# rust-av/grav1synth

Measured on AMD Instinct MI355X. Metric: diff Mpixels/s (luma pixels of frame pairs fully processed: flat-block finder + AR accumulation + block stats + ordered fold), higher is better.
Workload: dtype i8 x i8 -> i32 matrix-core products, i64 sums (exact integers) + f64 flat-block features

## Files before the change

grav1synth_amd/csrc/latest.hip:

```cpp
#include "latest_dev.h"

#include "fold.h"

#include <stdio.h>

namespace g1s {
namespace {

constexpr int kT = 512, kWaves = kT / 64;
constexpr int kChunk = 1024, kRounds = kChunk / kT;
constexpr double kTinyD = 1.0e-16;
constexpr double kNorm2D = 255.0 * 255.0;
constexpr int kNL = 2 * kNumBins;
constexpr int kArenaD = 2 * kChunk + 8 * kNumBins + 8, kArenaL = kChunk + 8 * kNumBins + 8, kArenaT = kChunk + 8;
static_assert(kNumBins == 20 && kMaxN == 25, "latest.hip: the solvers' static sizes");

struct Shared {
  alignas(16) double D[kArenaD];
  double Lw[kArenaL];
  double Bv[2][kArenaD];
  double Tv[2][kArenaT];
  uint16_t cnt[kRounds][kWaves][kNL];
  uint32_t beg[kNL], end[kNL];
  double arx[3][kMaxN + 1];
  double gain[3];
  long long nobs[3];
  int ar_ok[3];
  double diag[kNumBins], low[kNumBins], bsum[2][kNumBins], total[2];
  double sb[2][kNumBins], sx[2][kNumBins];
  int st_ok[2];
  double luma_x[kNumBins];
  uint32_t ne;
  uint32_t wsum[kWaves];
};

__device__ __forceinline__ double readlane_f64(double v, int j) {
  const unsigned long long u = (unsigned long long)__double_as_longlong(v);
  const uint32_t lo = (uint32_t)__builtin_amdgcn_readlane((int)(uint32_t)u, j), hi = (uint32_t)__builtin_amdgcn_readlane((int)(uint32_t)(u >> 32), j);
  return __longlong_as_double((long long)(((unsigned long long)hi << 32) | lo));
}
__device__ __forceinline__ int uniform(int v) { return __builtin_amdgcn_readfirstlane(v); }

template <int NMAX>
__device__ __forceinline__ bool wave_gauss(const int n, double (&a)[NMAX], double b, double (&x)[NMAX], const int lane) {
  int rap = lane;
  bool done = false, ok = true;
#pragma unroll
  for (int k = 0; k < NMAX - 1; ++k) {
    if (k < n - 1 && ok) {
      const double ck = fabs(a[k]);
      double cp = __shfl(ck, rap, 64);
      if (lane < k || lane >= n) cp = -1.0;
      double val = cp;
      int idx = lane;
#pragma unroll
      for (int d = 1; d < 32; d <<= 1) {
        const double v2 = __shfl_down(val, d, 64);
        const int i2 = __shfl_down(idx, d, 64);
        if (lane + d < 64 && v2 > val) {
          val = v2;
          idx = i2;
        }
      }
      const int rap_w = __shfl(rap, idx, 64);
      const int rap_up = __shfl_up(rap, 1, 64);
      const double cp_up = __shfl_up(cp, 1, 64);
      if (lane >= k && lane < n) rap = (lane == k) ? rap_w : ((cp_up < val) ? rap_up : rap_w);
      const int pr = uniform(__shfl(rap, k, 64));
      const double pk = readlane_f64(a[k], pr), bk = readlane_f64(b, pr);
      if (fabs(pk) < kTinyD) {
        ok = false;
      } else {
        if (lane == pr) done = true;
        const bool active = lane < n && !done;
        const double c = a[k] / pk;
#pragma unroll
        for (int j = k + 1; j < NMAX; ++j) {
          const double pj = readlane_f64(a[j], pr);
          const double t = c * pj;
          if (active && j < n) a[j] = a[j] - t;
        }
        const double t = c * bk;
        if (active) b = b - t;
      }
    }
  }
#pragma unroll
  for (int i = NMAX - 1; i >= 0; --i) {
    if (i < n && ok) {
      const int r = uniform(__shfl(rap, i, 64));
      const double piv = readlane_f64(a[i], r);
      if (fabs(piv) < kTinyD) {
        ok = false;
      } else {
        double c = 0;
#pragma unroll
        for (int j = i + 1; j < NMAX; ++j) {
          const double t = a[j] * x[j];
          if (j < n) c += t;
        }
        const double xi = (b - c) / a[i];
        x[i] = __shfl(xi, r, 64);
      }
    }
  }
  return ok;
}

__device__ inline double dev_clamp(double v, double lo, double hi) { return v < lo ? lo : (v > hi ? hi : v); }
__device__ inline double dev_bin_index(double value) { return (kNumBins - 1) * dev_clamp(value, 0.0, 255.0) / 255.0; }

__device__ __forceinline__ double div_count(double v, int count) {
  return (count & (count - 1)) == 0 ? __builtin_ldexp(v, -__builtin_ctz((unsigned)count)) : v / count;
}

__device__ inline void put_text(char *dst, const char *msg) {
  int i = 0;
  for (; msg[i] && i < 103; ++i) dst[i] = msg[i];
  dst[i] = 0;
}

#ifdef G1S_LATEST_TIMERS
#define K4_TICK(slot)                                 \
  do {                                                \
    __syncthreads();                                  \
    if (tid == 0 && frame == 0) {                     \
      const unsigned long long now_ = wall_clock64(); \
      k4_dbg[slot] += (double)(now_ - k4_t);          \
      k4_t = now_;                                    \
    }                                                 \
  } while (0)
#else
#define K4_TICK(slot) \
  do {                \
  } while (0)
#endif

struct FrameCtx {
  const uint8_t *rec;
  const uint8_t *mask;
  const uint32_t *luma_sum;
  int nb, nbw, W, H;
};

template <int NP>
__device__ __forceinline__ void strength_pass(Shared &sh, const LatestJob &job, const FrameCtx &fc, const int c0, const int tid, double *k4_dbg, const int frame) {
#ifdef G1S_LATEST_TIMERS
  unsigned long long k4_t = wall_clock64();
#endif
  const int lane = tid & 63, wave = tid >> 6;
  const bool is_chroma = c0 != 0;
  const int sx = is_chroma ? job.xdec : 0, sy = is_chroma ? job.ydec : 0;
  const int bw = kBlock >> sx, bh = kBlock >> sy;
  const int pw = job.W >> sx, ph = job.H >> sy;
  const int32_t *sum_d[NP];
  const uint32_t *sum_d2[NP];
  double noise_gain[NP], corr[NP];
#pragma unroll
  for (int q = 0; q < NP; ++q) {
    sum_d[q] = reinterpret_cast<const int32_t *>(fc.rec + job.L.off_sum_d[c0 + q]);
    sum_d2[q] = reinterpret_cast<const uint32_t *>(fc.rec + job.L.off_sum_d2[c0 + q]);
    noise_gain[q] = sh.gain[c0 + q];
    corr[q] = is_chroma ? sh.arx[c0 + q][job.n] : 0;
  }
  const double luma_gain = sh.gain[0];
  double acc = 0;
  uint32_t ne = 0;

  struct Raw {
    uint32_t m, ls;
    int32_t sd[NP];
    uint32_t sd2[NP];
  };
  Raw nxt[kRounds];
  auto fetch = [&](int base) {
#pragma unroll
    for (int r = 0; r < kRounds; ++r) {
      const int bi = base + kT * r + tid;
      const bool in = bi < fc.nb;
      nxt[r].m = in ? fc.mask[bi] : 0u;
      nxt[r].ls = in ? fc.luma_sum[bi] : 0u;
#pragma unroll
      for (int q = 0; q < NP; ++q) {
        nxt[r].sd[q] = in ? sum_d[q][bi] : 0;
        nxt[r].sd2[q] = in ? sum_d2[q][bi] : 0u;
      }
    }
  };
  fetch(0);
  for (int base = 0; base < fc.nb; base += kChunk) {
    Raw cur[kRounds];
#pragma unroll
    for (int r = 0; r < kRounds; ++r) cur[r] = nxt[r];
    if (base + kChunk < fc.nb) fetch(base + kChunk);
    int key[kRounds];
    double tU[kRounds], tW[kRounds], tV[kRounds], tP[kRounds][NP], tQ[kRounds][NP], tS[kRounds][NP];
#pragma unroll
    for (int r = 0; r < kRounds; ++r) {
      const int bi = base + kT * r + tid;
      key[r] = -1;
      tU[r] = tW[r] = tV[r] = 0;
#pragma unroll
      for (int q = 0; q < NP; ++q) tP[r][q] = tQ[r][q] = tS[r][q] = 0;
      if (cur[r].m == 0) continue;
      const int by = bi / fc.nbw, bx = bi - by * fc.nbw;
      const int shh = min(ph - by * bh, bh), sw = min(pw - bx * bw, bw);
      if (!(sw * shh > kBlock)) continue;
      const int lw = min(fc.W - bx * kBlock, kBlock), lh = min(fc.H - by * kBlock, kBlock);
      const double block_mean = div_count((double)cur[r].ls, lw * lh);
      const double bin = dev_bin_index(block_mean);
      const int i0 = (int)bin;
      const int i1 = min(kNumBins - 1, i0 + 1);
      const double a = bin - i0;
      key[r] = i0;
      tU[r] = (1.0 - a) * (1.0 - a);
      tW[r] = a * (1.0 - a);
      tV[r] = a * a;
      const double luma_strength = is_chroma ? luma_gain * ((1.0 - a) * sh.luma_x[i0] + a * sh.luma_x[i1]) : 0;
#pragma unroll
      for (int q = 0; q < NP; ++q) {
        double noise_mean = (double)cur[r].sd[q];
        const double noise_sq = (double)cur[r].sd2[q];
        noise_mean = div_count(noise_mean, sw * shh);
        const double noise_var = div_count(noise_sq, sw * shh) - noise_mean * noise_mean;
        const double cl = corr[q] * luma_strength;
        const double t0 = noise_var / 16, t1 = noise_var - cl * cl;
        const double uncorr_std = sqrt(t0 > t1 ? t0 : t1);
        const double noise_std = uncorr_std / noise_gain[q];
        tS[r][q] = noise_std;
        tP[r][q] = (1.0 - a) * noise_std;
        tQ[r][q] = a * noise_std;
      }
    }
    K4_TICK(6);
    uint32_t rk_own[kRounds], rk_prev[kRounds], rk_low[kRounds], rk_all[kRounds];
#pragma unroll
    for (int r = 0; r < kRounds; ++r) {
      unsigned long long prevB = 0;
      uint32_t mycnt = 0;
      rk_own[r] = rk_prev[r] = rk_low[r] = rk_all[r] = 0;
      const int kk = key[r];
#pragma unroll
      for (int k = 0; k < kNumBins; ++k) {
        const unsigned long long Bk = __ballot(kk == k);
        const unsigned long long M = Bk | prevB;
        if (M == 0) continue;
        const uint32_t preM = __builtin_amdgcn_mbcnt_hi((uint32_t)(M >> 32), __builtin_amdgcn_mbcnt_lo((uint32_t)M, 0u));
        const uint32_t preB = __builtin_amdgcn_mbcnt_hi((uint32_t)(Bk >> 32), __builtin_amdgcn_mbcnt_lo((uint32_t)Bk, 0u));
        if (kk == k) rk_own[r] = preM, rk_low[r] = preB;
        if (kk == k - 1) rk_prev[r] = preM;
        if (lane == k) mycnt = (uint32_t)__popcll(M);
        if (lane == kNumBins + k) mycnt = (uint32_t)__popcll(Bk);
        prevB = Bk;
      }
      {
        const unsigned long long Ma = __ballot(kk >= 0);
        rk_all[r] = __builtin_amdgcn_mbcnt_hi((uint32_t)(Ma >> 32), __builtin_amdgcn_mbcnt_lo((uint32_t)Ma, 0u));
        if (lane == kNL - 1) mycnt = (uint32_t)__popcll(Ma);
      }
      if (lane < kNL) sh.cnt[r][wave][lane] = (uint16_t)mycnt;
    }
    __syncthreads();
    K4_TICK(7);
    uint32_t my_off[kRounds];
    uint32_t run = 0;
#pragma unroll
    for (int r = 0; r < kRounds; ++r) my_off[r] = 0;
    if (lane < kNL) {
#pragma unroll
      for (int r = 0; r < kRounds; ++r)
#pragma unroll
        for (int w = 0; w < kWaves; ++w) {
          if (w == wave) my_off[r] = run;
          run += sh.cnt[r][w][lane];
        }
    }
    {
      const uint32_t room = (run + 7u) & ~7u;
      uint32_t incl = room;
#pragma unroll
      for (int d = 1; d < 64; d <<= 1) {
        const uint32_t o = (uint32_t)__shfl_up((int)incl, d, 64);
        if (lane >= d) incl += o;
      }
      const uint32_t upto19 = (uint32_t)__shfl((int)incl, kNumBins - 1, 64);
      uint32_t bse = incl - room;
      if (lane >= kNumBins) bse -= upto19;
      if (lane == kNL - 1) bse = 0;
#pragma unroll
      for (int r = 0; r < kRounds; ++r) my_off[r] += bse;
      if (wave == 0 && lane < kNL) {
        sh.beg[lane] = bse;
        sh.end[lane] = bse + run;
        if (lane < kNumBins) {
          for (uint32_t i = bse + run; i < bse + room; ++i) {
            sh.D[i] = 0.0;
#pragma unroll
            for (int q = 0; q < NP; ++q) sh.Bv[q][i] = 0.0;
          }
        } else if (lane < kNL - 1) {
          for (uint32_t i = bse + run; i < bse + room; ++i) sh.Lw[i] = 0.0;
        } else {
          for (uint32_t i = run; i < room; ++i) {
#pragma unroll
            for (int q = 0; q < NP; ++q) sh.Tv[q][i] = 0.0;
          }
        }
      }
    }
    K4_TICK(8);
#pragma unroll
    for (int r = 0; r < kRounds; ++r) {
      const int kk = key[r], kq = max(kk, 0);
      const uint32_t o_own = (uint32_t)__shfl((int)my_off[r], kq, 64);
      const uint32_t o_prev = (uint32_t)__shfl((int)my_off[r], min(kq + 1, kNumBins - 1), 64);
      const uint32_t o_low = (uint32_t)__shfl((int)my_off[r], kNumBins + min(kq, kNumBins - 2), 64);
      const uint32_t o_all = (uint32_t)__shfl((int)my_off[r], kNL - 1, 64);
      if (kk < 0) continue;
      const uint32_t so = o_own + rk_own[r];
      sh.D[so] = tU[r];
#pragma unroll
      for (int q = 0; q < NP; ++q) sh.Bv[q][so] = tP[r][q];
      if (kk < kNumBins - 1) {
        const uint32_t sp = o_prev + rk_prev[r];
        sh.D[sp] = tV[r];
#pragma unroll
        for (int q = 0; q < NP; ++q) sh.Bv[q][sp] = tQ[r][q];
        const uint32_t sl = o_low + rk_low[r];
        sh.Lw[sl] = tW[r];
      }
      const uint32_t st = o_all + rk_all[r];
#pragma unroll
      for (int q = 0; q < NP; ++q) sh.Tv[q][st] = tS[r][q];
    }
    __syncthreads();
    K4_TICK(9);
    if (wave == 0 || wave == 2) {
      constexpr int kLowLanes = kNumBins - 1;
      const int arr = wave == 0 ? lane / kNumBins : (lane < kLowLanes ? 3 : 4 + (lane - kLowLanes));
      const int li = wave == 0 ? lane % kNumBins : (lane < kLowLanes ? kNumBins + lane : kNL - 1);
      const bool on = wave == 0 ? arr <= NP : lane < kLowLanes + NP;
      const double2 *src = reinterpret_cast<const double2 *>(arr == 0 ? sh.D : arr == 1 ? sh.Bv[0] : arr == 2 ? sh.Bv[NP - 1] : arr == 3 ? sh.Lw : arr == 4 ? sh.Tv[0] : sh.Tv[NP - 1]);
      if (on) {
        uint32_t i = sh.beg[li] >> 1;
        const uint32_t e = (sh.end[li] + 1) >> 1;
        double2 va[4], vb[4];
#pragma unroll
        for (int u = 0; u < 4; ++u) va[u] = src[i + u];
        while (i < e) {
#pragma unroll
          for (int u = 0; u < 4; ++u) vb[u] = src[i + 4 + u];
#pragma unroll
          for (int u = 0; u < 4; ++u) acc += va[u].x, acc += va[u].y;
          i += 4;
          if (i < e) {
#pragma unroll
            for (int u = 0; u < 4; ++u) va[u] = src[i + 4 + u];
#pragma unroll
            for (int u = 0; u < 4; ++u) acc += vb[u].x, acc += vb[u].y;
            i += 4;
          }
        }
        if (wave == 2 && lane == kLowLanes) ne += sh.end[kNL - 1];
      }
    }
    __syncthreads();
    K4_TICK(10);
  }
  if (wave == 0) {
    const int k = lane % kNumBins, arr = lane / kNumBins;
    if (arr == 0) sh.diag[k] = acc;
    else if (arr <= NP) sh.bsum[arr - 1][k] = acc;
  } else if (wave == 2) {
    if (lane < kNumBins - 1) sh.low[lane] = acc;
    else if (lane < kNumBins - 1 + NP) sh.total[lane - (kNumBins - 1)] = acc;
    if (lane == kNumBins - 1) sh.ne = ne;
  }
  __syncthreads();
}

__device__ __forceinline__ void strength_solve(Shared &sh, const int q, const int lane) {
  const uint32_t ne = sh.ne;
  double r[kNumBins], x[kNumBins];
  const int i = lane < kNumBins ? lane : 0, nn = kNumBins;
  const double mean = sh.total[q] / (int)ne;
  const double sb = sh.bsum[q][i] + mean / 8192.;
  const double alpha = 2.0 * (double)(int)ne / nn;
  const int lo = max(0, i - 1), hi = min(nn - 1, i + 1);
#pragma unroll
  for (int j = 0; j < kNumBins; ++j) {
    double v = 0.0;
    if (i == j) v = sh.diag[i];
    else if (i == j + 1) v = sh.low[j];
    else if (j == i + 1) v = sh.low[i];
    r[j] = v;
    x[j] = 0.0;
  }
#pragma unroll
  for (int j = 0; j < kNumBins; ++j)
    if (j == lo) r[j] -= alpha;
#pragma unroll
  for (int j = 0; j < kNumBins; ++j)
    if (j == i) r[j] += 2 * alpha;
#pragma unroll
  for (int j = 0; j < kNumBins; ++j)
    if (j == hi) r[j] -= alpha;
#pragma unroll
  for (int j = 0; j < kNumBins; ++j)
    if (j == i) r[j] += 1.0 / 8192.;
  const bool ok = wave_gauss<kNumBins>(kNumBins, r, sb, x, lane);
  if (lane < kNumBins) {
    sh.sb[q][lane] = sb;
    double xv = 0.0;
#pragma unroll
    for (int j = 0; j < kNumBins; ++j)
      if (j == lane) xv = x[j];
    sh.sx[q][lane] = xv;
  }
  if (lane == 0) sh.st_ok[q] = ok ? 1 : 0;
}

__global__ __launch_bounds__(kT) void k4_latest(LatestJob job) {
  __shared__ Shared sh;
  const int tid = threadIdx.x, lane = tid & 63, wave = tid >> 6, frame = blockIdx.x;
  const uint8_t *rec = job.records + job.L.size * (size_t)frame;
  uint8_t *blob = job.blobs + job.blob_bytes * (size_t)frame;
  const int nb = (int)job.L.nblocks;
  const int n = job.n, ncm = n + 1;
  FrameCtx fc;
  fc.rec = rec;
  fc.mask = rec + job.L.off_mask;
  fc.luma_sum = reinterpret_cast<const uint32_t *>(rec + job.L.off_luma_sum);
  fc.nb = nb;
  fc.nbw = job.nbw;
  fc.W = job.W;
  fc.H = job.H;

  double *k4_dbg = reinterpret_cast<double *>(job.scratch);
#ifdef G1S_LATEST_TIMERS
  unsigned long long k4_t = wall_clock64();
  if (tid < 16 && frame == 0) k4_dbg[tid] = 0.0;
  __syncthreads();
#endif
  for (size_t k = tid; k < job.blob_bytes / 8; k += kT) reinterpret_cast<unsigned long long *>(blob)[k] = 0ull;
  LatestHeader *hdr = reinterpret_cast<LatestHeader *>(blob);
  auto plane_head = [&](int c) { return reinterpret_cast<LatestPlaneHead *>(blob + sizeof(LatestHeader) + c * plane_blob_bytes(ncm)); };
  auto plane_doubles = [&](int c) { return reinterpret_cast<double *>(blob + sizeof(LatestHeader) + c * plane_blob_bytes(ncm) + sizeof(LatestPlaneHead)); };
  uint32_t nflat_t = 0;
  for (int b = tid; b < nb; b += kT) nflat_t += fc.mask[b] != 0;
#pragma unroll
  for (int d = 32; d > 0; d >>= 1) nflat_t += (uint32_t)__shfl_down((int)nflat_t, d, 64);
  if (lane == 0) sh.wsum[wave] = nflat_t;
  __syncthreads();
  uint32_t num_flat = 0;
#pragma unroll
  for (int w = 0; w < kWaves; ++w) num_flat += sh.wsum[w];
  if (tid == 0) {
    hdr->magic = kLatestMagic;
    hdr->lag = (uint32_t)job.lag;
    hdr->nplanes = (uint32_t)job.nplanes;
    hdr->status = G1S_OK;
    hdr->size_bytes = (uint32_t)job.blob_bytes;
    hdr->reserved = num_flat;
    for (int c = 0; c < 3; ++c) plane_head(c)->ar_gain = 1.0;
  }
  if (num_flat <= 1) {
    if (tid == 0) {
      hdr->status = G1S_ERR_NOT_ENOUGH_FLAT;
      put_text(hdr->err, "Not enough flat blocks to update noise estimate");
    }
    return;
  }
  K4_TICK(0);

  auto ar_entry = [&](int c, int i, int j) -> double {
    const bool is_chroma = c != 0;
    const int nc = n + (is_chroma ? 1 : 0);
    const int64_t *S = reinterpret_cast<const int64_t *>(rec + job.L.off_ar[c]);
    const double ns = is_chroma ? (double)((1 << job.xdec) * (1 << job.ydec)) : 1.0;
    double den = kNorm2D;
    if (is_chroma && i == nc - 1) den *= ns;
    if (is_chroma && j == nc - 1) den *= ns;
    const int64_t s = j == nc ? S[(size_t)nc * nc + i] : (i <= j ? S[i * nc + j] : S[j * nc + i]);
    return (double)s / den;
  };
  if (wave < job.nplanes) {
    const int c = wave;
    const bool is_chroma = c != 0;
    const int nc = n + (is_chroma ? 1 : 0);
    const int row = lane < nc ? lane : 0;
    double a[kMaxN], x[kMaxN];
#pragma unroll
    for (int j = 0; j < kMaxN; ++j) {
      a[j] = j < nc ? ar_entry(c, row, j) : 0.0;
      x[j] = 0.0;
    }
    const double b0 = ar_entry(c, row, nc);
    const double a_diag = ar_entry(c, row, row), a_last = ar_entry(c, row, nc - 1);
    const int64_t nobs = reinterpret_cast<const int64_t *>(rec + job.L.off_ar[c])[(size_t)nc * nc + nc];
    const bool ok = wave_gauss<kMaxN>(nc, a, b0, x, lane);
    double gain = 1.0;
    if (ok) {
      const int m = nc - (is_chroma ? 1 : 0);
      double x_mine = 0.0;
#pragma unroll
      for (int j = 0; j < kMaxN; ++j)
        if (j == lane) x_mine = x[j];
      const double tv = a_diag / nobs;
      double bi = b0, x_last = 0.0;
#pragma unroll
      for (int j = 0; j < kMaxN; ++j)
        if (j == nc - 1) x_last = x[j];
      if (is_chroma) bi -= a_last * x_last;
      const double tc = (bi * x_mine) / nobs;
      double var = 0, sum_covar = 0;
      for (int i = 0; i < m; ++i) var += readlane_f64(tv, i);
      var /= m;
      for (int i = 0; i < m; ++i) sum_covar += readlane_f64(tc, i);
      const double t = var - sum_covar;
      const double noise_var = t > 1e-6 ? t : 1e-6;
      const double q = var / noise_var;
      const double g = sqrt(q > 1e-6 ? q : 1e-6);
      gain = 1 > g ? 1 : g;
    } else if (is_chroma) {
      const int last = nc - 1;
      const double all = readlane_f64(a_diag, last), bl = readlane_f64(b0, last);
#pragma unroll
      for (int j = 0; j < kMaxN; ++j) x[j] = 0.0;
      if (fabs(all) > 1e-6) {
        const double xl = bl / all;
#pragma unroll
        for (int j = 0; j < kMaxN; ++j)
          if (j == last) x[j] = xl;
      }
    }
    if (lane < nc) {
      double xv = 0.0;
#pragma unroll
      for (int j = 0; j < kMaxN; ++j)
        if (j == lane) xv = x[j];
      sh.arx[c][lane] = xv;
    }
    if (lane == 0) {
      sh.gain[c] = gain;
      sh.nobs[c] = nobs;
      sh.ar_ok[c] = ok ? 1 : 0;
    }
  }
  __syncthreads();
  K4_TICK(1);
  auto write_ar = [&](int c) {
    const bool is_chroma = c != 0;
    const int nc = n + (is_chroma ? 1 : 0);
    double *pd = plane_doubles(c);
    for (int e = tid; e < nc * nc + nc; e += kT) {
      if (e < nc * nc) {
        const int i = e / nc, j = e - i * nc;
        pd[e] = ar_entry(c, i, j);
      } else {
        const int i = e - nc * nc;
        pd[ncm * ncm + i] = ar_entry(c, i, nc);
        pd[ncm * ncm + ncm + i] = sh.arx[c][i];
      }
    }
    if (tid == 0) {
      LatestPlaneHead *ph = plane_head(c);
      ph->num_observations = sh.nobs[c];
      ph->ar_gain = sh.gain[c];
    }
  };
  auto write_strength = [&](int c, int q) {
    double *qd = plane_doubles(c) + ncm * ncm + 2 * ncm;
    for (int e = tid; e < kNumBins * kNumBins; e += kT) {
      const int i = e / kNumBins, j = e - i * kNumBins;
      double v = 0.0;
      if (i == j) v = sh.diag[i];
      else if (i == j + 1) v = sh.low[j];
      else if (j == i + 1) v = sh.low[i];
      qd[e] = v;
    }
    if (tid < kNumBins) {
      qd[kNumBins * kNumBins + tid] = sh.sb[q][tid];
      qd[kNumBins * kNumBins + kNumBins + tid] = sh.sx[q][tid];
    }
    if (tid == 0) {
      LatestPlaneHead *ph = plane_head(c);
      ph->num_equations = (int32_t)sh.ne;
      ph->total = sh.total[q];
    }
  };
  write_ar(0);
  if (!sh.ar_ok[0]) {
    if (tid == 0) {
      hdr->status = G1S_ERR_SOLVE;
      put_text(hdr->err, "Solving latest noise equation system failed 0!");
    }
    return;
  }
  strength_pass<1>(sh, job, fc, 0, tid, k4_dbg, frame);
  K4_TICK(2);
  if (wave == 0) strength_solve(sh, 0, lane);
  __syncthreads();
  write_strength(0, 0);
  if (tid < kNumBins) sh.luma_x[tid] = sh.sx[0][tid];
  if (!sh.st_ok[0]) {
    if (tid == 0) {
      hdr->status = G1S_ERR_SOLVE;
      put_text(hdr->err, "Solving latest noise strength failed!");
    }
    return;
  }
  __syncthreads();
  K4_TICK(3);
  if (job.nplanes < 3) return;
  strength_pass<2>(sh, job, fc, 1, tid, k4_dbg, frame);
  K4_TICK(4);
  if (wave < 2) strength_solve(sh, wave, lane);
  __syncthreads();
  write_ar(1);
  write_strength(1, 0);
  if (!sh.st_ok[0]) {
    if (tid == 0) {
      hdr->status = G1S_ERR_SOLVE;
      put_text(hdr->err, "Solving latest noise strength failed!");
    }
    return;
  }
  write_ar(2);
  write_strength(2, 1);
  if (!sh.st_ok[1]) {
    if (tid == 0) {
      hdr->status = G1S_ERR_SOLVE;
      put_text(hdr->err, "Solving latest noise strength failed!");
    }
  }
  K4_TICK(5);
}

}

size_t latest_scratch_bytes(uint32_t) { return 256; }
const char *latest_kernel_name() { return "k4_latest"; }

hipError_t launch_latest(const LatestJob &job, int frames, hipStream_t stream) {
  if (frames <= 0) return hipSuccess;
  hipLaunchKernelGGL(k4_latest, dim3(frames), dim3(kT), 0, stream, job);
#ifdef G1S_LATEST_TIMERS
  {
    double t[16];
    (void)hipStreamSynchronize(stream);
    (void)hipMemcpy(t, job.scratch, sizeof(t), hipMemcpyDeviceToHost);
    fprintf(stderr, "k4_latest phases, us (frame 0): head %.1f  ar solves %.1f  luma pass %.1f  luma solve %.1f  chroma pass %.1f  chroma solves %.1f | inside both passes: "
                    "terms %.1f  ranks %.1f  offsets %.1f  scatter %.1f  chains %.1f\n",
            t[0] / 100, t[1] / 100, t[2] / 100, t[3] / 100, t[4] / 100, t[5] / 100, t[6] / 100, t[7] / 100, t[8] / 100, t[9] / 100, t[10] / 100);
  }
#endif
  return hipGetLastError();
}

}
```

Baseline: 657,200.

## Pipeline strength pass with dedicated chain waves and double-buffered arenas; DPP pivot search

Splits the block into 8 producer waves and 2 extra high-priority chain waves. Producers compute terms and ranks for stage t+2 and scatter stage t+1 into double-buffered shared arenas while the chain waves sum stage t, so each stage needs one barrier instead of two. The stage size drops from 1024 to 512 blocks. The Gaussian pivot argmax now uses DPP row shifts and readlane in place of shfl_down/shfl, which caps the system size at 32. The cost is more threads per block, a larger shared-memory footprint, and more pipeline stages for the same work.

```diff
diff --git a/grav1synth_amd/csrc/latest.hip b/grav1synth_amd/csrc/latest.hip
--- a/grav1synth_amd/csrc/latest.hip
+++ b/grav1synth_amd/csrc/latest.hip
@@ -7,21 +7,24 @@
 namespace g1s {
 namespace {
 
-constexpr int kT = 512, kWaves = kT / 64;
-constexpr int kChunk = 1024, kRounds = kChunk / kT;
+constexpr int kPT = 512, kPW = kPT / 64;
+constexpr int kCW = 2;
+constexpr int kT = kPT + 64 * kCW, kWaves = kT / 64;
+constexpr int kStage = 512, kRounds = kStage / kPT;
 constexpr double kTinyD = 1.0e-16;
 constexpr double kNorm2D = 255.0 * 255.0;
 constexpr int kNL = 2 * kNumBins;
-constexpr int kArenaD = 2 * kChunk + 8 * kNumBins + 8, kArenaL = kChunk + 8 * kNumBins + 8, kArenaT = kChunk + 8;
+constexpr int kArenaD = 2 * kStage + 8 * kNumBins + 8, kArenaL = kStage + 8 * kNumBins + 8, kArenaT = kStage + 8;
 static_assert(kNumBins == 20 && kMaxN == 25, "latest.hip: the solvers' static sizes");
+static_assert(kArenaD % 2 == 0 && kArenaL % 2 == 0 && kArenaT % 2 == 0, "latest.hip: the chains read the arenas as double2");
 
 struct Shared {
-  alignas(16) double D[kArenaD];
-  double Lw[kArenaL];
-  double Bv[2][kArenaD];
-  double Tv[2][kArenaT];
-  uint16_t cnt[kRounds][kWaves][kNL];
-  uint32_t beg[kNL], end[kNL];
+  alignas(16) double D[2][kArenaD];
+  double Lw[2][kArenaL];
+  double Bv[2][2][kArenaD];
+  double Tv[2][2][kArenaT];
+  uint16_t cnt[2][kRounds][kPW][kNL];
+  uint32_t beg[2][kNL], end[2][kNL];
   double arx[3][kMaxN + 1];
   double gain[3];
   long long nobs[3];
@@ -39,10 +42,30 @@
   const uint32_t lo = (uint32_t)__builtin_amdgcn_readlane((int)(uint32_t)u, j), hi = (uint32_t)__builtin_amdgcn_readlane((int)(uint32_t)(u >> 32), j);
   return __longlong_as_double((long long)(((unsigned long long)hi << 32) | lo));
 }
-__device__ __forceinline__ int uniform(int v) { return __builtin_amdgcn_readfirstlane(v); }
+
+template <int CTRL>
+__device__ __forceinline__ int dpp_i32(int old, int v) {
+  return __builtin_amdgcn_update_dpp(old, v, CTRL, 0xf, 0xf, false);
+}
+template <int CTRL>
+__device__ __forceinline__ double dpp_f64(double old, double v) {
+  const unsigned long long u = (unsigned long long)__double_as_longlong(v), o = (unsigned long long)__double_as_longlong(old);
+  const uint32_t lo = (uint32_t)dpp_i32<CTRL>((int)(uint32_t)o, (int)(uint32_t)u), hi = (uint32_t)dpp_i32<CTRL>((int)(uint32_t)(o >> 32), (int)(uint32_t)(u >> 32));
+  return __longlong_as_double((long long)(((unsigned long long)hi << 32) | lo));
+}
+template <int D>
+__device__ __forceinline__ void argmax_step(double &val, int &idx) {
+  const double v2 = dpp_f64<0x100 + D>(-1.0, val);
+  const int i2 = dpp_i32<0x100 + D>(0, idx);
+  if (v2 > val) {
+    val = v2;
+    idx = i2;
+  }
+}
 
 template <int NMAX>
 __device__ __forceinline__ bool wave_gauss(const int n, double (&a)[NMAX], double b, double (&x)[NMAX], const int lane) {
+  static_assert(NMAX <= 32, "wave_gauss: the pivot search covers two rows of 16 lanes");
   int rap = lane;
   bool done = false, ok = true;
 #pragma unroll
@@ -53,20 +76,23 @@
       if (lane < k || lane >= n) cp = -1.0;
       double val = cp;
       int idx = lane;
-#pragma unroll
-      for (int d = 1; d < 32; d <<= 1) {
-        const double v2 = __shfl_down(val, d, 64);
-        const int i2 = __shfl_down(idx, d, 64);
-        if (lane + d < 64 && v2 > val) {
+      argmax_step<1>(val, idx);
+      argmax_step<2>(val, idx);
+      argmax_step<4>(val, idx);
+      argmax_step<8>(val, idx);
+      {
+        const double v2 = readlane_f64(val, 16);
+        const int i2 = __builtin_amdgcn_readlane(idx, 16);
+        if (lane < 16 && v2 > val) {
           val = v2;
           idx = i2;
         }
       }
       const int rap_w = __shfl(rap, idx, 64);
-      const int rap_up = __shfl_up(rap, 1, 64);
-      const double cp_up = __shfl_up(cp, 1, 64);
+      const int rap_up = dpp_i32<0x138>(0, rap);
+      const double cp_up = dpp_f64<0x138>(-1.0, cp);
       if (lane >= k && lane < n) rap = (lane == k) ? rap_w : ((cp_up < val) ? rap_up : rap_w);
-      const int pr = uniform(__shfl(rap, k, 64));
+      const int pr = __builtin_amdgcn_readlane(rap, k);
       const double pk = readlane_f64(a[k], pr), bk = readlane_f64(b, pr);
       if (fabs(pk) < kTinyD) {
         ok = false;
@@ -88,7 +114,7 @@
 #pragma unroll
   for (int i = NMAX - 1; i >= 0; --i) {
     if (i < n && ok) {
-      const int r = uniform(__shfl(rap, i, 64));
+      const int r = __builtin_amdgcn_readlane(rap, i);
       const double piv = readlane_f64(a[i], r);
       if (fabs(piv) < kTinyD) {
         ok = false;
@@ -100,7 +126,7 @@
           if (j < n) c += t;
         }
         const double xi = (b - c) / a[i];
-        x[i] = __shfl(xi, r, 64);
+        x[i] = readlane_f64(xi, r);
       }
     }
   }
@@ -130,9 +156,17 @@
       k4_t = now_;                                    \
     }                                                 \
   } while (0)
+#define K4_BUSY_BEGIN() const unsigned long long busy_t_ = wall_clock64()
+#define K4_BUSY_END(var) (var) += wall_clock64() - busy_t_
 #else
 #define K4_TICK(slot) \
   do {                \
+  } while (0)
+#define K4_BUSY_BEGIN() \
+  do {                  \
+  } while (0)
+#define K4_BUSY_END(var) \
+  do {                   \
   } while (0)
 #endif
 
@@ -145,10 +179,9 @@
 
 template <int NP>
 __device__ __forceinline__ void strength_pass(Shared &sh, const LatestJob &job, const FrameCtx &fc, const int c0, const int tid, double *k4_dbg, const int frame) {
-#ifdef G1S_LATEST_TIMERS
-  unsigned long long k4_t = wall_clock64();
-#endif
   const int lane = tid & 63, wave = tid >> 6;
+  const bool chain_wave = wave >= kPW;
+  const int cw = wave - kPW;
   const bool is_chroma = c0 != 0;
   const int sx = is_chroma ? job.xdec : 0, sy = is_chroma ? job.ydec : 0;
   const int bw = kBlock >> sx, bh = kBlock >> sy;
@@ -164,8 +197,20 @@
     corr[q] = is_chroma ? sh.arx[c0 + q][job.n] : 0;
   }
   const double luma_gain = sh.gain[0];
+  const int stages = (fc.nb + kStage - 1) / kStage;
+#ifdef G1S_LATEST_TIMERS
+  unsigned long long busy_place = 0, busy_measure = 0, busy_chain = 0;
+#endif
+
+  constexpr int kLowLanes = kNumBins - 1;
+  const int arr = cw == 0 ? lane / kNumBins : (lane < kLowLanes ? 3 : 4 + (lane - kLowLanes));
+  const int li = cw == 0 ? lane % kNumBins : (lane < kLowLanes ? kNumBins + lane : kNL - 1);
+  const bool on = chain_wave && (cw == 0 ? arr <= NP : lane < kLowLanes + NP);
+  const double2 *const src0 = reinterpret_cast<const double2 *>(arr == 0 ? sh.D[0] : arr == 1 ? sh.Bv[0][0] : arr == 2 ? sh.Bv[0][NP - 1] : arr == 3 ? sh.Lw[0] : arr == 4 ? sh.Tv[0][0] : sh.Tv[0][NP - 1]);
+  const uint32_t buf_stride = (arr == 0 ? kArenaD : arr <= 2 ? 2 * kArenaD : arr == 3 ? kArenaL : 2 * kArenaT) / 2;
   double acc = 0;
   uint32_t ne = 0;
+  if (chain_wave) __builtin_amdgcn_s_setprio(3);
 
   struct Raw {
     uint32_t m, ls;
@@ -176,7 +221,7 @@
   auto fetch = [&](int base) {
 #pragma unroll
     for (int r = 0; r < kRounds; ++r) {
-      const int bi = base + kT * r + tid;
+      const int bi = base + kPT * r + tid;
       const bool in = bi < fc.nb;
       nxt[r].m = in ? fc.mask[bi] : 0u;
       nxt[r].ls = in ? fc.luma_sum[bi] : 0u;
@@ -187,163 +232,175 @@
       }
     }
   };
-  fetch(0);
-  for (int base = 0; base < fc.nb; base += kChunk) {
-    Raw cur[kRounds];
-#pragma unroll
-    for (int r = 0; r < kRounds; ++r) cur[r] = nxt[r];
-    if (base + kChunk < fc.nb) fetch(base + kChunk);
-    int key[kRounds];
-    double tU[kRounds], tW[kRounds], tV[kRounds], tP[kRounds][NP], tQ[kRounds][NP], tS[kRounds][NP];
-#pragma unroll
-    for (int r = 0; r < kRounds; ++r) {
-      const int bi = base + kT * r + tid;
-      key[r] = -1;
-      tU[r] = tW[r] = tV[r] = 0;
-#pragma unroll
-      for (int q = 0; q < NP; ++q) tP[r][q] = tQ[r][q] = tS[r][q] = 0;
-      if (cur[r].m == 0) continue;
-      const int by = bi / fc.nbw, bx = bi - by * fc.nbw;
-      const int shh = min(ph - by * bh, bh), sw = min(pw - bx * bw, bw);
-      if (!(sw * shh > kBlock)) continue;
-      const int lw = min(fc.W - bx * kBlock, kBlock), lh = min(fc.H - by * kBlock, kBlock);
-      const double block_mean = div_count((double)cur[r].ls, lw * lh);
-      const double bin = dev_bin_index(block_mean);
-      const int i0 = (int)bin;
-      const int i1 = min(kNumBins - 1, i0 + 1);
-      const double a = bin - i0;
-      key[r] = i0;
-      tU[r] = (1.0 - a) * (1.0 - a);
-      tW[r] = a * (1.0 - a);
-      tV[r] = a * a;
-      const double luma_strength = is_chroma ? luma_gain * ((1.0 - a) * sh.luma_x[i0] + a * sh.luma_x[i1]) : 0;
-#pragma unroll
-      for (int q = 0; q < NP; ++q) {
-        double noise_mean = (double)cur[r].sd[q];
-        const double noise_sq = (double)cur[r].sd2[q];
-        noise_mean = div_count(noise_mean, sw * shh);
-        const double noise_var = div_count(noise_sq, sw * shh) - noise_mean * noise_mean;
-        const double cl = corr[q] * luma_strength;
-        const double t0 = noise_var / 16, t1 = noise_var - cl * cl;
-        const double uncorr_std = sqrt(t0 > t1 ? t0 : t1);
-        const double noise_std = uncorr_std / noise_gain[q];
-        tS[r][q] = noise_std;
-        tP[r][q] = (1.0 - a) * noise_std;
-        tQ[r][q] = a * noise_std;
-      }
-    }
-    K4_TICK(6);
-    uint32_t rk_own[kRounds], rk_prev[kRounds], rk_low[kRounds], rk_all[kRounds];
-#pragma unroll
-    for (int r = 0; r < kRounds; ++r) {
-      unsigned long long prevB = 0;
-      uint32_t mycnt = 0;
-      rk_own[r] = rk_prev[r] = rk_low[r] = rk_all[r] = 0;
-      const int kk = key[r];
-#pragma unroll
-      for (int k = 0; k < kNumBins; ++k) {
-        const unsigned long long Bk = __ballot(kk == k);
-        const unsigned long long M = Bk | prevB;
-        if (M == 0) continue;
-        const uint32_t preM = __builtin_amdgcn_mbcnt_hi((uint32_t)(M >> 32), __builtin_amdgcn_mbcnt_lo((uint32_t)M, 0u));
-        const uint32_t preB = __builtin_amdgcn_mbcnt_hi((uint32_t)(Bk >> 32), __builtin_amdgcn_mbcnt_lo((uint32_t)Bk, 0u));
-        if (kk == k) rk_own[r] = preM, rk_low[r] = preB;
-        if (kk == k - 1) rk_prev[r] = preM;
-        if (lane == k) mycnt = (uint32_t)__popcll(M);
-        if (lane == kNumBins + k) mycnt = (uint32_t)__popcll(Bk);
-        prevB = Bk;
-      }
-      {
-        const unsigned long long Ma = __ballot(kk >= 0);
-        rk_all[r] = __builtin_amdgcn_mbcnt_hi((uint32_t)(Ma >> 32), __builtin_amdgcn_mbcnt_lo((uint32_t)Ma, 0u));
-        if (lane == kNL - 1) mycnt = (uint32_t)__popcll(Ma);
-      }
-      if (lane < kNL) sh.cnt[r][wave][lane] = (uint16_t)mycnt;
-    }
-    __syncthreads();
-    K4_TICK(7);
-    uint32_t my_off[kRounds];
-    uint32_t run = 0;
-#pragma unroll
-    for (int r = 0; r < kRounds; ++r) my_off[r] = 0;
-    if (lane < kNL) {
-#pragma unroll
-      for (int r = 0; r < kRounds; ++r)
-#pragma unroll
-        for (int w = 0; w < kWaves; ++w) {
-          if (w == wave) my_off[r] = run;
-          run += sh.cnt[r][w][lane];
-        }
-    }
-    {
-      const uint32_t room = (run + 7u) & ~7u;
-      uint32_t incl = room;
-#pragma unroll
-      for (int d = 1; d < 64; d <<= 1) {
-        const uint32_t o = (uint32_t)__shfl_up((int)incl, d, 64);
-        if (lane >= d) incl += o;
-      }
-      const uint32_t upto19 = (uint32_t)__shfl((int)incl, kNumBins - 1, 64);
-      uint32_t bse = incl - room;
-      if (lane >= kNumBins) bse -= upto19;
-      if (lane == kNL - 1) bse = 0;
-#pragma unroll
-      for (int r = 0; r < kRounds; ++r) my_off[r] += bse;
-      if (wave == 0 && lane < kNL) {
-        sh.beg[lane] = bse;
-        sh.end[lane] = bse + run;
-        if (lane < kNumBins) {
-          for (uint32_t i = bse + run; i < bse + room; ++i) {
-            sh.D[i] = 0.0;
-#pragma unroll
-            for (int q = 0; q < NP; ++q) sh.Bv[q][i] = 0.0;
+  int key[kRounds];
+  double tU[kRounds], tW[kRounds], tV[kRounds], tP[kRounds][NP], tQ[kRounds][NP], tS[kRounds][NP];
+  uint32_t rk_own[kRounds], rk_prev[kRounds], rk_low[kRounds], rk_all[kRounds];
+#pragma unroll
+  for (int r = 0; r < kRounds; ++r) {
+    key[r] = -1;
+    tU[r] = tW[r] = tV[r] = 0;
+    rk_own[r] = rk_prev[r] = rk_low[r] = rk_all[r] = 0;
+#pragma unroll
+    for (int q = 0; q < NP; ++q) tP[r][q] = tQ[r][q] = tS[r][q] = 0;
+  }
+  if (!chain_wave) fetch(0);
+
+  for (int t = -2; t < stages; ++t) {
+    if (!chain_wave) {
+      if (t >= -1 && t + 1 < stages) {
+        K4_BUSY_BEGIN();
+        const int pb = (t + 1) & 1;
+        uint32_t my_off[kRounds];
+        uint32_t run = 0;
+#pragma unroll
+        for (int r = 0; r < kRounds; ++r) my_off[r] = 0;
+        if (lane < kNL) {
+#pragma unroll
+          for (int r = 0; r < kRounds; ++r)
+#pragma unroll
+            for (int w = 0; w < kPW; ++w) {
+              if (w == wave) my_off[r] = run;
+              run += sh.cnt[pb][r][w][lane];
+            }
+        }
+        {
+          const uint32_t room = (run + 7u) & ~7u;
+          uint32_t incl = room;
+#pragma unroll
+          for (int d = 1; d < 64; d <<= 1) {
+            const uint32_t o = (uint32_t)__shfl_up((int)incl, d, 64);
+            if (lane >= d) incl += o;
           }
-        } else if (lane < kNL - 1) {
-          for (uint32_t i = bse + run; i < bse + room; ++i) sh.Lw[i] = 0.0;
-        } else {
-          for (uint32_t i = run; i < room; ++i) {
-#pragma unroll
-            for (int q = 0; q < NP; ++q) sh.Tv[q][i] = 0.0;
+          const uint32_t upto19 = (uint32_t)__shfl((int)incl, kNumBins - 1, 64);
+          uint32_t bse = incl - room;
+          if (lane >= kNumBins) bse -= upto19;
+          if (lane == kNL - 1) bse = 0;
+#pragma unroll
+          for (int r = 0; r < kRounds; ++r) my_off[r] += bse;
+          if (wave == 0 && lane < kNL) {
+            sh.beg[pb][lane] = bse;
+            sh.end[pb][lane] = bse + run;
+            if (lane < kNumBins) {
+              for (uint32_t i = bse + run; i < bse + room; ++i) {
+                sh.D[pb][i] = 0.0;
+#pragma unroll
+                for (int q = 0; q < NP; ++q) sh.Bv[pb][q][i] = 0.0;
+              }
+            } else if (lane < kNL - 1) {
+              for (uint32_t i = bse + run; i < bse + room; ++i) sh.Lw[pb][i] = 0.0;
+            } else {
+              for (uint32_t i = run; i < room; ++i) {
+#pragma unroll
+                for (int q = 0; q < NP; ++q) sh.Tv[pb][q][i] = 0.0;
+              }
+            }
           }
         }
-      }
-    }
-    K4_TICK(8);
-#pragma unroll
-    for (int r = 0; r < kRounds; ++r) {
-      const int kk = key[r], kq = max(kk, 0);
-      const uint32_t o_own = (uint32_t)__shfl((int)my_off[r], kq, 64);
-      const uint32_t o_prev = (uint32_t)__shfl((int)my_off[r], min(kq + 1, kNumBins - 1), 64);
-      const uint32_t o_low = (uint32_t)__shfl((int)my_off[r], kNumBins + min(kq, kNumBins - 2), 64);
-      const uint32_t o_all = (uint32_t)__shfl((int)my_off[r], kNL - 1, 64);
-      if (kk < 0) continue;
-      const uint32_t so = o_own + rk_own[r];
-      sh.D[so] = tU[r];
-#pragma unroll
-      for (int q = 0; q < NP; ++q) sh.Bv[q][so] = tP[r][q];
-      if (kk < kNumBins - 1) {
-        const uint32_t sp = o_prev + rk_prev[r];
-        sh.D[sp] = tV[r];
-#pragma unroll
-        for (int q = 0; q < NP; ++q) sh.Bv[q][sp] = tQ[r][q];
-        const uint32_t sl = o_low + rk_low[r];
-        sh.Lw[sl] = tW[r];
-      }
-      const uint32_t st = o_all + rk_all[r];
-#pragma unroll
-      for (int q = 0; q < NP; ++q) sh.Tv[q][st] = tS[r][q];
-    }
-    __syncthreads();
-    K4_TICK(9);
-    if (wave == 0 || wave == 2) {
-      constexpr int kLowLanes = kNumBins - 1;
-      const int arr = wave == 0 ? lane / kNumBins : (lane < kLowLanes ? 3 : 4 + (lane - kLowLanes));
-      const int li = wave == 0 ? lane % kNumBins : (lane < kLowLanes ? kNumBins + lane : kNL - 1);
-      const bool on = wave == 0 ? arr <= NP : lane < kLowLanes + NP;
-      const double2 *src = reinterpret_cast<const double2 *>(arr == 0 ? sh.D : arr == 1 ? sh.Bv[0] : arr == 2 ? sh.Bv[NP - 1] : arr == 3 ? sh.Lw : arr == 4 ? sh.Tv[0] : sh.Tv[NP - 1]);
+#pragma unroll
+        for (int r = 0; r < kRounds; ++r) {
+          const int kk = key[r], kq = max(kk, 0);
+          const uint32_t o_own = (uint32_t)__shfl((int)my_off[r], kq, 64);
+          const uint32_t o_prev = (uint32_t)__shfl((int)my_off[r], min(kq + 1, kNumBins - 1), 64);
+          const uint32_t o_low = (uint32_t)__shfl((int)my_off[r], kNumBins + min(kq, kNumBins - 2), 64);
+          const uint32_t o_all = (uint32_t)__shfl((int)my_off[r], kNL - 1, 64);
+          if (kk < 0) continue;
+          const uint32_t so = o_own + rk_own[r];
+          sh.D[pb][so] = tU[r];
+#pragma unroll
+          for (int q = 0; q < NP; ++q) sh.Bv[pb][q][so] = tP[r][q];
+          if (kk < kNumBins - 1) {
+            const uint32_t sp = o_prev + rk_prev[r];
+            sh.D[pb][sp] = tV[r];
+#pragma unroll
+            for (int q = 0; q < NP; ++q) sh.Bv[pb][q][sp] = tQ[r][q];
+            const uint32_t sl = o_low + rk_low[r];
+            sh.Lw[pb][sl] = tW[r];
+          }
+          const uint32_t st = o_all + rk_all[r];
+#pragma unroll
+          for (int q = 0; q < NP; ++q) sh.Tv[pb][q][st] = tS[r][q];
+        }
+        K4_BUSY_END(busy_place);
+      }
+      if (t + 2 < stages) {
+        K4_BUSY_BEGIN();
+        const int base = (t + 2) * kStage, cb = t & 1;
+        Raw cur[kRounds];
+#pragma unroll
+        for (int r = 0; r < kRounds; ++r) cur[r] = nxt[r];
+        if (base + kStage < fc.nb) fetch(base + kStage);
+#pragma unroll
+        for (int r = 0; r < kRounds; ++r) {
+          const int bi = base + kPT * r + tid;
+          key[r] = -1;
+          tU[r] = tW[r] = tV[r] = 0;
+#pragma unroll
+          for (int q = 0; q < NP; ++q) tP[r][q] = tQ[r][q] = tS[r][q] = 0;
+          if (cur[r].m == 0) continue;
+          const int by = bi / fc.nbw, bx = bi - by * fc.nbw;
+          const int shh = min(ph - by * bh, bh), sw = min(pw - bx * bw, bw);
+          if (!(sw * shh > kBlock)) continue;
+          const int lw = min(fc.W - bx * kBlock, kBlock), lh = min(fc.H - by * kBlock, kBlock);
+          const double block_mean = div_count((double)cur[r].ls, lw * lh);
+          const double bin = dev_bin_index(block_mean);
+          const int i0 = (int)bin;
+          const int i1 = min(kNumBins - 1, i0 + 1);
+          const double a = bin - i0;
+          key[r] = i0;
+          tU[r] = (1.0 - a) * (1.0 - a);
+          tW[r] = a * (1.0 - a);
+          tV[r] = a * a;
+          const double luma_strength = is_chroma ? luma_gain * ((1.0 - a) * sh.luma_x[i0] + a * sh.luma_x[i1]) : 0;
+#pragma unroll
+          for (int q = 0; q < NP; ++q) {
+            double noise_mean = (double)cur[r].sd[q];
+            const double noise_sq = (double)cur[r].sd2[q];
+            noise_mean = div_count(noise_mean, sw * shh);
+            const double noise_var = div_count(noise_sq, sw * shh) - noise_mean * noise_mean;
+            const double cl = corr[q] * luma_strength;
+            const double t0 = noise_var / 16, t1 = noise_var - cl * cl;
+            const double uncorr_std = sqrt(t0 > t1 ? t0 : t1);
+            const double noise_std = uncorr_std / noise_gain[q];
+            tS[r][q] = noise_std;
+            tP[r][q] = (1.0 - a) * noise_std;
+            tQ[r][q] = a * noise_std;
+          }
+        }
+#pragma unroll
+        for (int r = 0; r < kRounds; ++r) {
+          unsigned long long prevB = 0;
+          uint32_t mycnt = 0;
+          rk_own[r] = rk_prev[r] = rk_low[r] = rk_all[r] = 0;
+          const int kk = key[r];
+#pragma unroll
+          for (int k = 0; k < kNumBins; ++k) {
+            const unsigned long long Bk = __ballot(kk == k);
+            const unsigned long long M = Bk | prevB;
+            if (M == 0) continue;
+            const uint32_t preM = __builtin_amdgcn_mbcnt_hi((uint32_t)(M >> 32), __builtin_amdgcn_mbcnt_lo((uint32_t)M, 0u));
+            const uint32_t preB = __builtin_amdgcn_mbcnt_hi((uint32_t)(Bk >> 32), __builtin_amdgcn_mbcnt_lo((uint32_t)Bk, 0u));
+            if (kk == k) rk_own[r] = preM, rk_low[r] = preB;
+            if (kk == k - 1) rk_prev[r] = preM;
+            if (lane == k) mycnt = (uint32_t)__popcll(M);
+            if (lane == kNumBins + k) mycnt = (uint32_t)__popcll(Bk);
+            prevB = Bk;
+          }
+          {
+            const unsigned long long Ma = __ballot(kk >= 0);
+            rk_all[r] = __builtin_amdgcn_mbcnt_hi((uint32_t)(Ma >> 32), __builtin_amdgcn_mbcnt_lo((uint32_t)Ma, 0u));
+            if (lane == kNL - 1) mycnt = (uint32_t)__popcll(Ma);
+          }
+          if (lane < kNL) sh.cnt[cb][r][wave][lane] = (uint16_t)mycnt;
+        }
+        K4_BUSY_END(busy_measure);
+      }
+    } else if (t >= 0) {
+      K4_BUSY_BEGIN();
+      const int rb = t & 1;
       if (on) {
-        uint32_t i = sh.beg[li] >> 1;
-        const uint32_t e = (sh.end[li] + 1) >> 1;
+        const double2 *src = src0 + (rb ? buf_stride : 0u);
+        uint32_t i = sh.beg[rb][li] >> 1;
+        const uint32_t e = (sh.end[rb][li] + 1) >> 1;
         double2 va[4], vb[4];
 #pragma unroll
         for (int u = 0; u < 4; ++u) va[u] = src[i + u];
@@ -361,21 +418,28 @@
             i += 4;
           }
         }
-        if (wave == 2 && lane == kLowLanes) ne += sh.end[kNL - 1];
-      }
+        if (cw == 1 && lane == kLowLanes) ne += sh.end[rb][kNL - 1];
+      }
+      K4_BUSY_END(busy_chain);
     }
     __syncthreads();
-    K4_TICK(10);
-  }
-  if (wave == 0) {
-    const int k = lane % kNumBins, arr = lane / kNumBins;
+  }
+  if (chain_wave) __builtin_amdgcn_s_setprio(0);
+  if (chain_wave && cw == 0) {
+    const int k = lane % kNumBins;
     if (arr == 0) sh.diag[k] = acc;
     else if (arr <= NP) sh.bsum[arr - 1][k] = acc;
-  } else if (wave == 2) {
-    if (lane < kNumBins - 1) sh.low[lane] = acc;
-    else if (lane < kNumBins - 1 + NP) sh.total[lane - (kNumBins - 1)] = acc;
-    if (lane == kNumBins - 1) sh.ne = ne;
-  }
+  } else if (chain_wave) {
+    if (lane < kLowLanes) sh.low[lane] = acc;
+    else if (lane < kLowLanes + NP) sh.total[lane - kLowLanes] = acc;
+    if (lane == kLowLanes) sh.ne = ne;
+  }
+#ifdef G1S_LATEST_TIMERS
+  if (frame == 0 && lane == 0) {
+    if (wave == 0) k4_dbg[6] += (double)busy_measure, k4_dbg[7] += (double)busy_place;
+    if (chain_wave) k4_dbg[8 + cw] += (double)busy_chain;
+  }
+#endif
   __syncthreads();
 }
 
@@ -650,9 +714,9 @@
     double t[16];
     (void)hipStreamSynchronize(stream);
     (void)hipMemcpy(t, job.scratch, sizeof(t), hipMemcpyDeviceToHost);
-    fprintf(stderr, "k4_latest phases, us (frame 0): head %.1f  ar solves %.1f  luma pass %.1f  luma solve %.1f  chroma pass %.1f  chroma solves %.1f | inside both passes: "
-                    "terms %.1f  ranks %.1f  offsets %.1f  scatter %.1f  chains %.1f\n",
-            t[0] / 100, t[1] / 100, t[2] / 100, t[3] / 100, t[4] / 100, t[5] / 100, t[6] / 100, t[7] / 100, t[8] / 100, t[9] / 100, t[10] / 100);
+    fprintf(stderr, "k4_latest phases, us (frame 0): head %.1f  ar solves %.1f  luma pass %.1f  luma solve %.1f  chroma pass %.1f  chroma solves %.1f | busy inside both passes, each wave's own clock: "
+                    "wave 0 measure %.1f  place %.1f  chain wave 8 %.1f  chain wave 9 %.1f\n",
+            t[0] / 100, t[1] / 100, t[2] / 100, t[3] / 100, t[4] / 100, t[5] / 100, t[6] / 100, t[7] / 100, t[8] / 100, t[9] / 100);
   }
 #endif
   return hipGetLastError();
```

After: 670,200, median of 6. 1.02x the previous value.
